# termuxinator/html5-canvas-raytracer

Hardware: AMD Instinct MI355X
Metric: Mpixel/s (higher is better)
Workload: dtype f64; 1 GPU; cfg3: h8 scene (8 spheres, 2 lights, depth 3, supersample 1) at 3840x2160; SCENE, CAMERA AND LAUNCH TABLE RESIDENT (a static frame rendered again and again: cold_frame / new_camera_every_step are the other cases); one launch per frame; kernel=fma

## Files before the change

html5-canvas-raytracer_amd/csrc/rt_kernel_math.h:

```cpp

struct v3 { double x, y, z; };
__device__ __forceinline__ v3 mk(double x, double y, double z) { v3 r; r.x = x; r.y = y; r.z = z; return r; }
__device__ __forceinline__ double dot(const v3 a, const v3 b) { return a.x * b.x + a.y * b.y + a.z * b.z; }

#if RT_STRICT
__device__ __forceinline__ double rt_sqrt(double x) { return sqrt(x); }
template <bool FMIN = false> __device__ __forceinline__ double rt_sqrt_nn(double x) { return sqrt(x); }
__device__ __forceinline__ double rt_rcp(double x) { return 1.0 / x; }
__device__ __forceinline__ double rt_div(double a, double b) { return a / b; }
__device__ __forceinline__ double rt_pow(double x, double e) { return pow(x, e); }
#define RT_DIV_CONST(x, c) ((x) / (c))
__device__ __forceinline__ v3 unit(const v3 v, double *len_out) {
  const double l = sqrt(dot(v, v));
  *len_out = l;
  if (l != 0.0) { const double s = 1.0 / l; return mk(v.x * s, v.y * s, v.z * s); }
  return v;
}
#else
__device__ __forceinline__ double rt_rsqrt_pos(double m) {
  const double y = __builtin_amdgcn_rsq(m);
  const double e = __builtin_fma(-(m * y), y, 1.0);
  return __builtin_fma(0.5 * y, e, y);
}
__device__ __forceinline__ double rt_sqrt(double x) {
  const double y = rt_rsqrt_pos(x);
  double g = x * y;
  g = __builtin_fma(__builtin_fma(-g, g, x), 0.5 * y, g);
  return (x > 0.0) ? g : x;
}
template <bool FMIN = false>
__device__ __forceinline__ double rt_sqrt_nn(double x) {
  double y;
  if constexpr (FMIN) y = __builtin_fmin(__builtin_amdgcn_rsq(x), 1e100);
  else {
    const unsigned long long yb = __builtin_bit_cast(unsigned long long, __builtin_amdgcn_rsq(x));
    const int32_t yh = (int32_t)(yb >> 32);
    y = __builtin_bit_cast(double, ((unsigned long long)(uint32_t)(yh < 0x7fe00000 ? yh : 0x7fe00000) << 32) | (uint32_t)yb);
  }
  const double e = __builtin_fma(-(x * y), y, 1.0);
  y = __builtin_fma(0.5 * y, e, y);
  const double g = x * y;
  return __builtin_fma(__builtin_fma(-g, g, x), 0.5 * y, g);
}
__device__ __forceinline__ double rt_rcp(double x) {
  double y = __builtin_amdgcn_rcp(x);
  y = __builtin_fma(y, __builtin_fma(-x, y, 1.0), y);
  return __builtin_fma(y, __builtin_fma(-x, y, 1.0), y);
}
__device__ __forceinline__ double rt_div(double a, double b) {
  const double r = rt_rcp(b);
  const double q = a * r;
  return __builtin_fma(__builtin_fma(-q, b, a), r, q);
}
#define RT_DIV_CONST(x, c) rt_div_const((x), (c), 1.0 / (c))
__device__ __forceinline__ double rt_div_const(double a, double c, double rc) {
  const double q = a * rc;
  return __builtin_fma(__builtin_fma(-q, c, a), rc, q);
}
__device__ __attribute__((noinline)) double rt_pow_generic(double x, double e) { return pow(x, e); }
template <bool UNI = false, class EP>
__device__ __forceinline__ double rt_pow_spec(double x, int32_t n, EP e) {
  const int32_t n0 = UNI ? n : __builtin_amdgcn_readfirstlane(n);
  if (UNI || __ballot(n != n0) == 0ull) {
    if (n0 < 0) return rt_pow_generic(x, *e);
    uint32_t k = (uint32_t)n0;
    if (k == 0u) return 1.0;
    double b = x;
    uint32_t g = __builtin_ctz(k);
    for (uint32_t i = 0; i < g; i++) b *= b;
    double r = b;
    for (k >>= g + 1u; k != 0u; k >>= g + 1u) {
      g = __builtin_ctz(k);
      for (uint32_t i = 0; i <= g; i++) b *= b;
      r *= b;
    }
    return r;
  }
  if (n < 0) return rt_pow_generic(x, *e);
  double r = 1.0, b = x;
  uint32_t k = (uint32_t)n;
  do { if (k & 1u) r *= b; b *= b; k >>= 1; } while (__ballot(k != 0u) != 0ull);
  return r;
}
__device__ __forceinline__ v3 unit(const v3 v, double *len_out) {
  const double m = dot(v, v);
  const double s = rt_rsqrt_pos(m);
  const bool ok = (m > 0.0);
  *len_out = ok ? m * s : m;
  return ok ? mk(v.x * s, v.y * s, v.z * s) : v;
}
#endif

#if RT_STRICT
#include "rt_fdlibm.h"
template <bool FMIN = false> __device__ __forceinline__ void rt_atan2_asin(double y, double x, double w, double *at, double *as) { *at = fd_atan2(y, x); *as = fd_asin(w); }
#else
__device__ __forceinline__ double rt_fma_k(double a, double b, double k) {
  double r;
  asm("v_fma_f64 %0, %1, %2, %3" : "=v"(r) : "v"(a), "v"(b), "s"(k));
  return r;
}
typedef const double __attribute__((address_space(4))) *rt_trig_kptr;
typedef double __attribute__((ext_vector_type(4))) rt_d4;
#define RT_TRIG_AHEAD 2u
__constant__ unsigned long long RT_TRIG_BITS[32] = {
    0x3eeba404b5e68a13ull, 0xbf23e260bd3237f4ull, 0x3f4b2bb069efb384ull, 0xbf67952daf56de9bull,
    0x3f7d6d43a595c56full, 0xbf8c6ea4a57d9582ull, 0x3f967e295f08b19full, 0xbf9e9ae6fc27006aull,
    0x3fa2c15b5711927aull, 0x3fa059859fea6a70ull, 0xbfa59976e82d3ff0ull, 0xbf90a5a378a05eafull,
    0x3fa82d5d6ef28734ull, 0x3f94052137024d6aull, 0xbfaae5ce6a214619ull, 0x3f7ab3a098a70509ull,
    0x3fae1bb48427b883ull, 0x3f88ed60a300c8d2ull, 0xbfb110e48b207f05ull, 0x3f8c6fa84b77012bull,
    0x3fb3b13657b87036ull, 0x3f91c6c111dccb70ull, 0xbfb745d119378e4full, 0x3f96e89f0a0adacfull,
    0x3fbc71c717e1913cull, 0x3f9f1c72c668963full, 0xbfc2492492376b7dull, 0x3fa6db6db41ce4bdull,
    0x3fc99999999952ccull, 0x3fb333333336fd5bull, 0xbfd5555555555523ull, 0x3fc5555555555380ull};
template <bool FMIN = false>
__device__ __forceinline__ void rt_atan2_asin(double y, double x, double w, double *at, double *as) {
  rt_trig_kptr K = (rt_trig_kptr)(const void *)RT_TRIG_BITS;
  asm volatile("" : "+s"(K));
#define RT_TRIG_GROUP(I) (*(const rt_d4 __attribute__((address_space(4))) *)(K + 4 * (I)))
  rt_d4 g[8];
  g[0] = RT_TRIG_GROUP(0); g[1] = RT_TRIG_GROUP(1);
  const double ax = __builtin_fabs(x), ay = __builtin_fabs(y);
  const double hi = __builtin_fmax(ax, ay), lo = __builtin_fmin(ax, ay);
  const double q = rt_div(lo, hi);
  const double z = q * q;
  const double yw = __builtin_fabs(w);
  const double t = __builtin_fma(yw, -0.5, 0.5);
  const bool big = (yw >= 0.5);
  const double r = big ? t : w * w;
  g[2] = RT_TRIG_GROUP(2);
  double p = g[0][0];
  p = rt_fma_k(p, z, g[0][1]); p = rt_fma_k(p, z, g[0][2]); p = rt_fma_k(p, z, g[0][3]);
  g[3] = RT_TRIG_GROUP(3);
  p = rt_fma_k(p, z, g[1][0]); p = rt_fma_k(p, z, g[1][1]); p = rt_fma_k(p, z, g[1][2]); p = rt_fma_k(p, z, g[1][3]);
  double pa = 0.0;
#pragma unroll
  for (uint32_t i = 2; i < 8; i++) {
    if (i + RT_TRIG_AHEAD < 8u) g[i + RT_TRIG_AHEAD] = RT_TRIG_GROUP(i + RT_TRIG_AHEAD);
    p = rt_fma_k(p, z, g[i][0]);
    pa = (i == 2u) ? g[i][1] : rt_fma_k(pa, r, g[i][1]);
    p = rt_fma_k(p, z, g[i][2]);
    pa = rt_fma_k(pa, r, g[i][3]);
  }
#undef RT_TRIG_GROUP
  double a = __builtin_fma(q, z * p, q);
  a = (ay > ax) ? (M_PI / 2.0 - a) : a;
  const bool xneg = (__builtin_bit_cast(unsigned long long, x) >> 63) != 0;
  a = xneg ? (M_PI - a) : a;
  a = (hi == 0.0) ? (xneg ? M_PI : 0.0) : a;
  *at = __builtin_copysign(a, y);
  pa = pa * r;
  const double sq = big ? rt_sqrt_nn<FMIN>(t) : yw;
  const double ww = __builtin_fma(sq, pa, sq);
  double b = big ? __builtin_fma(-2.0, ww, M_PI / 2.0) : ww;
  b = (yw > 1.0) ? __builtin_nan("") : b;
  *as = __builtin_copysign(b, w);
}
#endif

__device__ __forceinline__ v3 reflect(const v3 v, const v3 n) {
  const double t = -(2.0 * dot(v, n));
  return mk(v.x + n.x * t, v.y + n.y * t, v.z + n.z * t);
}
__device__ __forceinline__ double min1(double x) { return (x > 1.0) ? 1.0 : x; }
__device__ __forceinline__ double maxa(double a, double x) { return (x < a) ? a : x; }

__device__ __forceinline__ uint32_t lowbias32(uint32_t x) {
  x ^= x >> 16; x *= 0x7feb352du; x ^= x >> 15; x *= 0x846ca68bu; x ^= x >> 16;
  return x;
}
__device__ __forceinline__ double star_uniform(uint32_t pix_lo, uint32_t pix_hi, uint32_t path, uint32_t mix) {
  return (double)lowbias32(pix_lo ^ lowbias32(path + 0x9e3779b9u * ((pix_hi ^ mix) + 1u))) * (1.0 / 4294967296.0);
}

__device__ __forceinline__ int to_int32_bit0(double x) {
  if (fabs(x) < 2147483648.0) return (int)x & 1;
  if (!(fabs(x) < RT_INF)) return 0;
  double t = trunc(x);
  if (fabs(t) >= 4294967296.0) t = t - floor(t / 4294967296.0) * 4294967296.0;
  return (int)((long long)t & 1);
}

__device__ __forceinline__ uint32_t to_byte(double c) {
#if RT_STRICT
  return (uint32_t)__builtin_rint(__builtin_fmin(__builtin_fmax(255.0 * c, 0.0), 255.0));
#else
  const double s = __builtin_fmin(__builtin_fmax(255.0 * c, 0.0), 255.0) + 6755399441055744.0;
  return (uint32_t)__builtin_bit_cast(unsigned long long, s);
#endif
}
```

html5-canvas-raytracer_amd/csrc/rt_kernel_trace.h:

```cpp

#define RT_PIN() asm volatile("")
#define RT_ROOT(TCA, DISC)                                                                    \
        const double thc_ = rt_sqrt_nn<REFRACT>(DISC);                                                 \
        const double t0_ = (TCA) - thc_, t1_ = (TCA) + thc_;                                  \
        const bool in_ = (t0_ < eps);                                                         \
        const double t_ = in_ ? t1_ : t0_;
#define RT_CAND(IDX, TCA, DISC)                                                               \
      if (!((DISC) < 0.0)) {                                                                  \
        RT_PIN();                                                                             \
        RT_ROOT(TCA, DISC)                                                                    \
        const bool closer_ = (t_ < ht) && !(t_ < eps);              \
        ht = closer_ ? t_ : ht;                                                               \
        hcode = closer_ ? ((int)(2u * (IDX)) + (in_ ? 1 : 0)) : hcode;                        \
      }
#define RT_GENERIC(IDX, G)                                                                    \
      {                                                                                       \
        const v3 Lv_ = mk((G).ox - p.x, (G).oy - p.y, (G).oz - p.z);                          \
        const double tca_ = dot(d, Lv_);                                                      \
        const double disc_ = (G).r2 - (dot(Lv_, Lv_) - tca_ * tca_);                          \
        RT_CAND(IDX, tca_, disc_)                                                             \
      }
#define RT_ANCHORED_DISC(G)                                                                   \
        const double tca_ = d.x * (G).ox + d.y * (G).oy + d.z * (G).oz;                       \
        const double disc_ = __builtin_fma(tca_, tca_, -(G).r2);
#define RT_ANCHORED(IDX, G)                                                                   \
      {                                                                                       \
        RT_ANCHORED_DISC(G)                                                                   \
        RT_CAND(IDX, tca_, disc_)                                                             \
      }

#if !RT_STRICT
__device__ __forceinline__ float rt_q_of(float qp, float x, float c, float rp_over_r) {
  const float ic = __builtin_amdgcn_rcpf(fmaxf(c, 1e-30f));
  return fminf(ic * (qp * (6.f * x + rp_over_r) + x + 0.5f * x * x) + x, 1e30f);
}
__device__ __forceinline__ int rt_lvl(int lv) { return lv & 255; }
#define RT_Q_GET(L_) __builtin_bit_cast(float, (uint32_t)(L_) & 0xffff0000u)
__device__ __forceinline__ int rt_q_put(int lv, float q) { return (int)(((uint32_t)lv & 0xffffu) | ((__builtin_bit_cast(uint32_t, q) + 0xffffu) & 0xffff0000u)); }
__device__ __forceinline__ float rt_r_get(int lv) { return __builtin_bit_cast(float, ((uint32_t)lv & 0xff00u) << 15); }
__device__ __forceinline__ int rt_r_put(int lv, float r) { return (int)(((uint32_t)lv & 0xffff00ffu) | ((((__builtin_bit_cast(uint32_t, r) >> 23) + 1u) & 255u) << 8)); }
constexpr float RT_Q_FLAT = 4096.f;
#define RT_Q_OF(QP, T, INVR, C, RP) rt_q_of((QP), (T) * (INVR), (C), (RP) * (INVR))
#else
__device__ __forceinline__ int rt_lvl(int lv) { return lv; }
#endif

#if !RT_STRICT
#define RT_XY_INDEX(XU, XV, FU, FV)                                                                                \
          const unsigned long long su = __builtin_bit_cast(unsigned long long, (XU) + 6442450944.0), sv = __builtin_bit_cast(unsigned long long, (XV) + 6442450944.0);   \
          uint32_t iu = __builtin_amdgcn_alignbit((uint32_t)(su >> 32), (uint32_t)su, 20u) ^ 0x80000000u;        \
          uint32_t iv = __builtin_amdgcn_alignbit((uint32_t)(sv >> 32), (uint32_t)sv, 20u) ^ 0x80000000u;       \
           \
          const bool near_ = (min(((uint32_t)su + 1u) & 0xfffffu, ((uint32_t)sv + 1u) & 0xfffffu) <= 2u);           \
           \
          if constexpr (UNI) { if (__ballot(near_) != 0ull) return false; }                                    \
          if (!UNI && near_) {                                                                                  \
            RT_PIN();                                                                                             \
            iu = (uint32_t)(XU); iv = (uint32_t)(XV);                    \
            const rt_launch __attribute__((address_space(4))) *K = rt_cold_args();                                \
             \
            float q_here = RT_Q_GET(level);                                                                        \
            if (rt_lvl(level) == 0 && q_here == 0.f) {                   \
              const float ex = (float)(h.x - K->cam_origin[0]), ey = (float)(h.y - K->cam_origin[1]), ez = (float)(h.z - K->cam_origin[2]);   \
              q_here = RT_Q_OF(0.f, __builtin_sqrtf(ex * ex + ey * ey + ez * ez), (float)m.inv_r, __builtin_fabsf((float)dot(d, n)), 0.f);       \
            }                                                                                                     \
            double tol = (K->mark_flags & RT_MARK_ALL) ? 2.0 : K->flag_tol * (double)fmaxf(1.f, q_here * (1.f / RT_Q_FLAT));   \
                          \
            if ((K->mark_flags & (RT_MARK_WEIGHT | RT_MARK_ALL)) == RT_MARK_WEIGHT) {                              \
              double S_ = map_valid ? acc[0] : 1.0;                                                               \
              if constexpr (FOLD_FORWARD && REFRACT) for (int i_ = 0; i_ < sp; i_++) S_ *= (parked[i_].map_valid ? parked[i_].S : 1.0) * parked[i_].a3;   \
              if (__builtin_fabs(S_) * 510.0 < 0.9) tol = -1.0;                                                    \
            }                                                                                                     \
             \
            const bool zf = !(K->mark_flags & RT_MARK_ZERO);                                                       \
            const bool bu = (zf && (FU) == 0.0 && (XU) == 0.0) || (__builtin_fabs((XU) - __builtin_rint(XU)) >= tol);    \
            const bool bv = (zf && (FV) == 0.0 && (XV) == 0.0) || (__builtin_fabs((XV) - __builtin_rint(XV)) >= tol);    \
            if (!(bu & bv)) {                                                                                      \
              uint32_t t3 = threadIdx.x;                                                                          \
              asm volatile("" : "+v"(t3));                                                                        \
              rt_mark_append<SS2>(rt_pixel_of<SS2, W1>(L, t3));                                                        \
            }                                                                                                     \
          }
#endif

#if !RT_STRICT
#define RT_SDISC(G, TC, DISC)                                                                 \
            const double TC = -(sv.x * (G).ox + sv.y * (G).oy + sv.z * (G).oz);               \
            const double DISC = __builtin_fma(TC, TC, -(G).r2);
#define RT_SROOTS(TC, THC, T0, T1) const double T0 = llen - (TC + THC), T1 = llen - (TC - THC);
#else
#define RT_SDISC(G, TC, DISC)                                                                 \
            const v3 Lv_ = mk((G).ox - h.x, (G).oy - h.y, (G).oz - h.z);                      \
            const double TC = dot(sv, Lv_);                                                   \
            const double DISC = (G).r2 - (dot(Lv_, Lv_) - TC * TC);
#define RT_SROOTS(TC, THC, T0, T1) const double T0 = TC - THC, T1 = TC + THC;
#endif
#define RT_SHADOW(J, G)                                                                       \
            {                                                                                 \
              const bool other_ = ((int)(J) != hi);                                           \
              if (COUNT && other_ && !blocked) tests++;                                       \
              RT_SDISC(G, tc_, disc_)                                                         \
              if (other_ && !(disc_ < 0.0) && !blocked) {                                     \
                RT_PIN();                                                                     \
                const double thc_ = rt_sqrt_nn<REFRACT>(disc_);                                        \
                RT_SROOTS(tc_, thc_, t0_, t1_)                                                \
                const double t_ = (t0_ < eps) ? t1_ : t0_;                                    \
                if ((t_ < llen) && !(t_ < eps)) {                                             \
                  RT_PIN();                                                                   \
                  const double oa4_ = objs[J].albedo[4];                                      \
                  if (oa4_ != 0.0) li = rt_div(li, oa4_);    \
                  else { li = 0.0; blocked = true; }                                          \
                }                                                                             \
              }                                                                               \
            }
#define RT_SHADOW_U(J, G)                                                                     \
            {                                                                               \
              RT_SDISC(G, tc_, disc_)                                                       \
              if (((int)(J) != hi) && !(disc_ < 0.0)) {                                     \
                RT_PIN();                                                                   \
                const double thc_ = rt_sqrt_nn<REFRACT>(disc_);                                      \
                RT_SROOTS(tc_, thc_, t0_, t1_)                                              \
                const double t_ = (t0_ < eps) ? t1_ : t0_;                                  \
                if ((t_ < llen) && !(t_ < eps) && li != 0.0) {                              \
                  RT_PIN();                                                                 \
                  const double oa4_ = objs[J].albedo[4];                                    \
                  li = (oa4_ != 0.0) ? rt_div(li, oa4_) : 0.0;                              \
                }                                                                           \
              }                                                                             \
            }

template <bool REFRACT, bool COUNT, bool GRID, bool SS2, bool ITEM = false, bool W1 = false, bool UNI = false>
__device__ __forceinline__ bool trace_pixel(const rt_launch &L, const rt_mtl *mtl, const rt_texture_desc *tex,
                                            [[maybe_unused]] double *acc, [[maybe_unused]] const rt_geom *cull_lds, [[maybe_unused]] const rt_geom cull0, [[maybe_unused]] uint32_t lane,
                                            [[maybe_unused]] double blk_x0, [[maybe_unused]] double blk_x1, [[maybe_unused]] double blk_y0,
                                            [[maybe_unused]] double blk_y1, v3 p, v3 d, double rgb[3], uint32_t cnt[3],
                                            [[maybe_unused]] bool is_probe, [[maybe_unused]] uint32_t cand_host,
                                            [[maybe_unused]] uint32_t own_sx = 0u, [[maybe_unused]] uint32_t own_sy = 0u, [[maybe_unused]] uint32_t own_f = 0u) {
  static_assert(!UNI || (W1 && !REFRACT && !COUNT && !ITEM && !RT_STRICT), "uniform-material path: the one-wave-workgroup product kernels");
#ifdef RT_TESTING
  uint32_t probe_n = 0;
  double probe_li = 0.0;
#endif
  const sphere_kptr objs = (sphere_kptr)L.objects;
  const geom_kptr geom = (geom_kptr)L.geom;
  const uint32_t N = L.n_objects, NL = L.n_lights;
  const double eps = L.epsilon;
  const uint32_t NLOOP = L.n_loop;
  const uint32_t enc = L.enclosing;
  const bool cull_lds_on = (!RT_STRICT && !COUNT) ? !GRID : (L.cull_in_lds != 0u);
#if RT_STRICT
  constexpr bool FOLD_FORWARD = false;
#else
  constexpr bool FOLD_FORWARD = true;
#endif
  [[maybe_unused]] frame<REFRACT> stack[FOLD_FORWARD ? 1 : RT_MAX_SEGS];
  [[maybe_unused]] park parked[(FOLD_FORWARD && REFRACT) ? RT_MAX_SEGS : 1];
  [[maybe_unused]] int sp = 0;
  [[maybe_unused]] bool map_valid = false;
  int level = 0;
  [[maybe_unused]] uint32_t tree_path = 1u;
#if defined(RT_TESTING) && defined(RT_ABLATE_BOUNCE)
  uint32_t segs_left = L.segs ? 1 : 0;
#else
  uint32_t segs_left = L.segs;
#endif
  double ret[3] = {0.0, 0.0, 0.0};

  double ht = RT_INF; int hcode = -1;
  if constexpr (UNI) { if (segs_left == 0) return false; }
  if (segs_left != 0) {
        [[maybe_unused]] const geom_kptr ga = (geom_kptr)L.geom_cam;
#if !RT_STRICT
        if constexpr (UNI) {
          const uint32_t i = cand_host & 255u;
          const rt_geom g0 = rt_load_geom32(ga, i);
          typename rt_mtl_src<true>::type &mu = *rt_mtl_at<true>(mtl, i);
          if ((mu.albedo[3] > 0.0 && segs_left > 1) || rt_mtl_kind(mu) == RT_SAMPLER_STARS) return false;
          RT_ANCHORED_DISC(g0)
          RT_ROOT(tca_, disc_)
          const bool met_ = !(disc_ < 0.0) && (t_ < ht) && !(t_ < eps);
          if (__ballot(!met_) != 0ull) return false;
#if defined(RT_TESTING) && defined(RT_ABLATE_UNIFORM)
          rgb[0] = rgb[1] = rgb[2] = 0.0;
          return true;
#endif
          ht = t_; hcode = (int)(2u * i) + (in_ ? 1 : 0);
        } else
        if (cand_host != 0u) {
          { const uint32_t i = cand_host & 255u; const rt_geom g0 = rt_load_geom32(ga, i); RT_ANCHORED(i, g0) }
          if (cand_host >= (2u << 16)) { const uint32_t i = (cand_host >> 8) & 255u; const rt_geom g0 = rt_load_geom32(ga, i); RT_ANCHORED(i, g0) }
        } else
#endif
        for (uint32_t base = 0; base < NLOOP; base += 64u) {
          const uint32_t j = base + lane;
          const uint32_t jj = j < NLOOP ? j : 0u;
          double c0 = cull0.ox, c1 = cull0.oy, c2 = cull0.oz, c3 = cull0.r2;
          if constexpr (ITEM) {
          } else if (cull_lds_on) {
            const rt_geom __attribute__((address_space(3))) *g = (const rt_geom __attribute__((address_space(3))) *)cull_lds + jj;
            c0 = g->ox; c1 = g->oy; c2 = g->oz; c3 = g->r2;
          } else if (base != 0u) {
            const rt_geom __attribute__((address_space(1))) *g = (const rt_geom __attribute__((address_space(1))) *)L.cull + jj;
            c0 = g->ox; c1 = g->oy; c2 = g->oz; c3 = g->r2;
          }
          const rt_geom cr = rt_geom{c0, c1, c2, c3};
          unsigned long long m = __ballot(j < NLOOP) & __ballot(cr.ox * L.proj_d <= blk_x1) & __ballot(cr.oy * L.proj_d >= blk_x0) &
                                 __ballot(cr.oz * L.proj_d <= blk_y1) & __ballot(cr.r2 * L.proj_d >= blk_y0);
          if constexpr (ITEM) m = (NLOOP - base >= 64u) ? ~0ull : ((1ull << (NLOOP - base)) - 1ull);
          while (m) {
            const uint32_t i = base + (uint32_t)__builtin_ctzll(m);
            m &= m - 1ull;
#if RT_STRICT
            const rt_geom g0 = rt_load_geom32(geom, i);
            RT_GENERIC(i, g0)
#else
            const rt_geom g0 = rt_load_geom32(ga, i);
            RT_ANCHORED(i, g0)
#endif
          }
        }
  }
  bool searched = true;
  [[maybe_unused]] bool first_bounce = false;
#if !RT_STRICT
  if (!UNI && L.sky_fast && segs_left != 0 && __ballot(hcode >= 0) == 0ull) {
    if (COUNT) { cnt[0]++; cnt[2] += N; }
    rgb[0] = L.sky_rgb[0]; rgb[1] = L.sky_rgb[1]; rgb[2] = L.sky_rgb[2];
    return true;
  }
#endif

  if (segs_left != 0) {
    for (;;) {
      if (COUNT) cnt[0]++;
      if (!UNI && !searched) {
        bool scanned = false;
#if !RT_STRICT
        if constexpr (GRID) {
          if (rt_cold_args()->bounce_table != nullptr) {
            const uint32_t from = (uint32_t)(hcode >> 1);
            const double ax = __builtin_fabs(d.x), ay = __builtin_fabs(d.y), az = __builtin_fabs(d.z);
            const bool bx = (ax >= ay) && (ax >= az), by = !bx && (ay >= az);
            const double dm = bx ? d.x : (by ? d.y : d.z);
            const double du = bx ? d.y : d.x, dv = (bx || by) ? d.z : d.y;
            const double sc = (0.5 * RT_BGRID) * __builtin_amdgcn_rcp(__builtin_fabs(dm));
            const double fu = __builtin_fmin(__builtin_fmax(__builtin_fma(du, sc, 0.5 * RT_BGRID), 0.0), (double)(RT_BGRID - 1u));
            const double fv = __builtin_fmin(__builtin_fmax(__builtin_fma(dv, sc, 0.5 * RT_BGRID), 0.0), (double)(RT_BGRID - 1u));
            const uint32_t face = (bx ? 0u : (by ? 2u : 4u)) + ((dm < 0.0) ? 1u : 0u);
            const uint32_t key = from * RT_BCELLS + face * (RT_BGRID * RT_BGRID) + (uint32_t)fv * RT_BGRID + (uint32_t)fu;
            const uint32_t words = (NLOOP + 63u) >> 6;
            ht = RT_INF; hcode = -1;
            for (uint32_t wd = 0; wd < words; wd++) {
              unsigned long long cand = 0ull, todo = __ballot(true);
              uint32_t distinct = 0;
              while (todo) {
                const uint32_t k0 = (uint32_t)__builtin_amdgcn_readlane((int)key, (int)__builtin_ctzll(todo));
                cand |= rt_load_word32(rt_cold_args()->bounce_table, k0 * words + wd);
                todo &= ~__ballot(key == k0);
                if (++distinct == 16u && todo) {
                  cand = (wd + 1u == words && (NLOOP & 63u)) ? ((1ull << (NLOOP & 63u)) - 1ull) : ~0ull;
                  break;
                }
              }
              while (cand) {
                const uint32_t j = (wd << 6) + (uint32_t)__builtin_ctzll(cand);
                cand &= cand - 1ull;
                const rt_geom g0 = rt_load_geom32(geom, j);
                RT_GENERIC(j, g0)
              }
            }
            scanned = true;
          }
        }
#endif
#if !RT_STRICT
        if constexpr (!GRID && !REFRACT && !COUNT && !ITEM) {
          if (first_bounce) {
            uint32_t fb = rt_entry_first_bounce<W1>(L);
#ifdef RT_TESTING
            if (L.no_first_bounce) fb = 0u;
#endif
            if (fb >> 31) {
              ht = RT_INF; hcode = -1;
              uint32_t m = (fb >> RT_CELL_SHIFT) & ((1u << RT_FB_MAX_LOOP) - 1u);
              uint32_t sn = rt_entry_second_node<W1>(L);
#ifdef RT_TESTING
              if (L.no_second_node) sn = 0u;
              if ((sn & (RT_SN_SELF0 | RT_SN_SELF1)) && L.uniform_waves != nullptr && __builtin_ctzll(__ballot(true)) == (int)lane) atomicAdd(L.uniform_waves + 3, 1ull);
#endif
              if (sn & RT_SN_SELF0) m &= ~(1u << (fb & 255u));
              if (sn & RT_SN_SELF1) m &= ~(1u << ((fb >> 8) & 255u));
              while (m) {
                const uint32_t i = (uint32_t)__builtin_ctz(m);
                m &= m - 1u;
                const rt_geom g0 = rt_load_geom32(geom, i);
                RT_GENERIC(i, g0)
              }
              scanned = true;
#ifdef RT_TESTING
              if (L.uniform_waves != nullptr && __builtin_ctzll(__ballot(true)) == (int)lane) atomicAdd(L.uniform_waves + 2, 1ull);
#endif
            }
          }
        }
#endif
        if (!scanned) {
          ht = RT_INF; hcode = -1;
          uint32_t i = 0;
          for (; i + 2 <= NLOOP; i += 2) {
            const rt_geom_pair gp = rt_load_geom_pair32(geom, i);
            const rt_geom g0 = gp.a, g1 = gp.b;
            RT_GENERIC(i, g0) RT_GENERIC(i + 1, g1)
          }
          if (i < NLOOP) { const rt_geom g0 = rt_load_geom32(geom, i); RT_GENERIC(i, g0) }
        }
      }
      [[maybe_unused]] const bool primary_node = UNI || searched;
      first_bounce = searched;
      searched = false;
      if (!UNI && enc != ~0u && hcode < 0) {
        if (L.enclosing_flat) {
          ht = 1.0; hcode = (int)(2u * enc + 1u);
        } else {
          const rt_geom g0 = rt_load_geom32(geom, enc);
          RT_GENERIC(enc, g0)
        }
      }
      if (COUNT) cnt[2] += N;
      const int hi = UNI ? (int)(cand_host & 255u) : (hcode >> 1);
      const bool inside = (hcode & 1) != 0;
      bool descend = false;
#if defined(RT_TESTING) && defined(RT_ABLATE_SHADE)
      if (true) { ret[0] = ht; ret[1] = (double)hcode; ret[2] = 0.0; } else
#endif
      if (!UNI && hcode < 0) {
        { const auto &mc = RT_COLD(miss_color); ret[0] = mc[0]; ret[1] = mc[1]; ret[2] = mc[2]; }
#ifdef RT_TESTING
        if (is_probe && probe_n < RT_PROBE_NODES) {
          double *q = L.probe + (size_t)(probe_n++) * RT_PROBE_WORDS;
          for (uint32_t z = 0; z < RT_PROBE_WORDS; z++) q[z] = 0.0;
          q[0] = (double)(REFRACT ? tree_path : (1u << rt_lvl(level))); q[1] = -1.0; q[2] = ht; q[9] = d.x; q[10] = d.y; q[11] = d.z;
          q[17] = (double)segs_left; q[19] = p.x; q[20] = p.y; q[21] = p.z; q[23] = 1.0;
        }
#endif
      } else {
        typename rt_mtl_src<UNI>::type &m = *rt_mtl_at<UNI>(mtl, (uint32_t)hi);
        const v3 h = mk(p.x + d.x * ht, p.y + d.y * ht, p.z + d.z * ht);
#if RT_STRICT
        double nlen;
        const v3 n = unit(mk(h.x - m.origin[0], h.y - m.origin[1], h.z - m.origin[2]), &nlen);
#else
        const double inv_r = m.inv_r;
        const v3 n = mk((h.x - m.origin[0]) * inv_r, (h.y - m.origin[1]) * inv_r, (h.z - m.origin[2]) * inv_r);
#endif
        v3 l;
        if (UNI && __ballot(inside) == 0ull) l = n;
        else l = inside ? mk(-n.x, -n.y, -n.z) : n;
        const double a0 = m.albedo[0], a1 = m.albedo[1], a2 = m.albedo[2], a3 = m.albedo[3];
        const double a4 = REFRACT ? m.albedo[4] : 0.0;
#if !RT_STRICT && !defined(RT_ABLATE_QAMP)
        if (!UNI && (rt_lvl(level) != 0 || ((a3 > 0.0 || a4 > 0.0) && segs_left > 1))) {
          const float ir_ = (float)inv_r;
          const float q_ = RT_Q_OF(RT_Q_GET(level), (float)ht, ir_, __builtin_fabsf((float)dot(d, n)), rt_r_get(level));
          level = rt_q_put(level, q_);
          level = rt_r_put(level, __builtin_amdgcn_rcpf(ir_));
        }
#endif

        double col[3];
#if defined(RT_TESTING) && defined(RT_ABLATE_SAMPLER)
        const int kind = RT_SAMPLER_COLOR;
#else
        const int kind = rt_mtl_kind(m);
#endif
#if RT_STRICT
        if (kind == RT_SAMPLER_TEXTURE) {
          double t_at, t_as;
          rt_atan2_asin<REFRACT>(-n.z, -n.x, -n.y, &t_at, &t_as);
          const double u = RT_DIV_CONST(t_at, M_PI) / 2.0 + 0.5;
          const double v = RT_DIV_CONST(t_as, M_PI / 2.0) / 2.0 + 0.5;
          const rt_texture_desc td = rt_tex_desc<UNI>(tex, rt_mtl_texture(m));
          const double xd = ceil(u * (double)td.width) - 1.0, yd = ceil(v * (double)td.height) - 1.0;
          uint32_t xi = (xd > 0.0) ? (uint32_t)xd : 0u, yi = (yd > 0.0) ? (uint32_t)yd : 0u;
          xi = min(xi, td.width - 1u); yi = min(yi, td.height - 1u);
          const uint32_t texel = *(const uint32_t *)(L.texel_base + td.texels_offset + ((size_t)yi * td.width + xi) * 4u);
          col[0] = RT_DIV_CONST((double)(texel & 255u), 255.0); col[1] = RT_DIV_CONST((double)((texel >> 8) & 255u), 255.0);
          col[2] = RT_DIV_CONST((double)((texel >> 16) & 255u), 255.0);
          if (xd != xd || yd != yd) col[0] = col[1] = col[2] = __builtin_nan("");
        } else if (kind == RT_SAMPLER_CHECKER) {
          double t_at, t_as;
          rt_atan2_asin<REFRACT>(-n.y, -n.x, -n.z, &t_at, &t_as);
          const double u = RT_DIV_CONST(t_at, M_PI) / 2.0 + 0.5;
          const double v = RT_DIV_CONST(t_as, M_PI / 2.0) / 2.0 + 0.5;
          const int c = to_int32_bit0(u * m.c[6]) ^ to_int32_bit0(v * m.c[7]);
          col[0] = m.c[3 * c]; col[1] = m.c[3 * c + 1]; col[2] = m.c[3 * c + 2];
#else
        [[maybe_unused]] double t_at, t_as;
        [[maybe_unused]] const bool one_cell = UNI && !GRID && kind == RT_SAMPLER_CHECKER && (cand_host & (1u << 24)) != 0u;
        if (UNI && one_cell) {
          const uint32_t c3 = (cand_host >> 28) & 1u ? 3u : 0u;
          col[0] = m.c[c3]; col[1] = m.c[c3 + 1u]; col[2] = m.c[c3 + 2u];
        } else if (UNI && kind != RT_SAMPLER_TEXTURE && kind != RT_SAMPLER_CHECKER) {
          col[0] = m.c[0]; col[1] = m.c[1]; col[2] = m.c[2];
        } else {
        if constexpr (UNI) {
          const bool tx_ = (kind == RT_SAMPLER_TEXTURE);
          rt_atan2_asin<REFRACT>(tx_ ? -n.z : -n.y, -n.x, tx_ ? -n.y : -n.z, &t_at, &t_as);
        }
        if (kind == RT_SAMPLER_TEXTURE) {
          if constexpr (!UNI) rt_atan2_asin<REFRACT>(-n.z, -n.x, -n.y, &t_at, &t_as);
          const double u = RT_DIV_CONST(t_at, M_PI) / 2.0 + 0.5;
          const double v = RT_DIV_CONST(t_as, M_PI / 2.0) / 2.0 + 0.5;
          const rt_texture_desc td = rt_tex_desc<UNI>(tex, rt_mtl_texture(m));
          const double xu = u * (double)td.width, xv = v * (double)td.height;
          RT_XY_INDEX(xu, xv, 1.0, 1.0)
          const uint32_t xi = min(iu, td.width - 1u), yi = min(iv, td.height - 1u);
          const uint32_t texel = *(const uint32_t *)(rt_cold_args()->texel_base + td.texels_offset + ((size_t)yi * td.width + xi) * 4u);
          col[0] = RT_DIV_CONST((double)(texel & 255u), 255.0); col[1] = RT_DIV_CONST((double)((texel >> 8) & 255u), 255.0);
          col[2] = RT_DIV_CONST((double)((texel >> 16) & 255u), 255.0);
        } else if (kind == RT_SAMPLER_CHECKER) {
          if constexpr (!UNI) rt_atan2_asin<REFRACT>(-n.y, -n.x, -n.z, &t_at, &t_as);
          const double u = RT_DIV_CONST(t_at, M_PI) / 2.0 + 0.5;
          const double v = RT_DIV_CONST(t_as, M_PI / 2.0) / 2.0 + 0.5;
          const double xu = u * m.c[6], xv = v * m.c[7];
          RT_XY_INDEX(xu, xv, m.c[6], m.c[7])
          const int c = (int)((iu ^ iv) & 1u);
          if constexpr (UNI) {
            double k0 = m.c[0], k1 = m.c[1], k2 = m.c[2], k3 = m.c[3], k4 = m.c[4], k5 = m.c[5];
            asm volatile("" : "+s"(k0), "+s"(k1), "+s"(k2), "+s"(k3), "+s"(k4), "+s"(k5));
            col[0] = c ? k3 : k0; col[1] = c ? k4 : k1; col[2] = c ? k5 : k2;
          } else { col[0] = m.c[3 * c]; col[1] = m.c[3 * c + 1]; col[2] = m.c[3 * c + 2]; }
#endif
        } else if (!UNI && kind == RT_SAMPLER_STARS) {
          uint32_t sx = own_sx, sy = own_sy, f = own_f;
          if constexpr (!ITEM) {
            f = blockIdx.z;
            uint32_t t3 = threadIdx.x;
            asm volatile("" : "+v"(t3));
            const rt_pixel P = rt_pixel_of<SS2, W1>(L, t3);
            sx = SS2 ? 2u * P.px + (P.sub & 1u) : P.px; sy = SS2 ? 2u * P.frow + (P.sub >> 1) : P.frow;
          }
          const unsigned long long pix = (unsigned long long)sy * (SS2 ? 2u * L.w : L.w) + sx;
          const uint32_t path = REFRACT ? tree_path : (1u << rt_lvl(level));
          const rt_launch __attribute__((address_space(4))) *K = rt_cold_args();
          const uint32_t mix = lowbias32(K->stars_seed + K->stars_step * f);
          double c = star_uniform((uint32_t)pix, (uint32_t)(pix >> 32), path, mix);
          c = (c >= m.c[6]) ? 0.0 : c * m.c[7];
          col[0] = col[1] = col[2] = c;
        } else { col[0] = m.c[0]; col[1] = m.c[1]; col[2] = m.c[2]; }
#if !RT_STRICT
        }
#endif

        if constexpr (FOLD_FORWARD && REFRACT) {
#pragma unroll
          for (int c = 0; c < 3; c++) acc[(10 + c) * RT_WG_THREADS] = col[c];
        }

        double diffuse = 0.0, specular = 0.0;
#if defined(RT_TESTING) && defined(RT_ABLATE_LIGHT)
        if (false) {
#else
        if (a1 > 0.0 || a2 > 0.0) {
#endif
          double li = RT_COLD(light_intensity);
#if !RT_STRICT
          [[maybe_unused]] uint32_t smask = ~0u;
          if constexpr (!COUNT) { if (primary_node) smask = rt_entry_shadow_masks<W1>(L); }
#endif
          for (uint32_t k = 0; k < NL; k++) {
            double llen;
            const double *lk = (const double *)((const char *)&L.lights[0][0] + (uint32_t)(k * 24u));
#if !RT_STRICT
            [[maybe_unused]] rt_geom_pair gp_first;
            if constexpr (!GRID && !COUNT) {
              [[maybe_unused]] const geom_kptr gl = (geom_kptr)L.geom_light;
              gp_first = rt_load_geom_pair32(gl, k * L.n_objects);
            }
#endif
            const v3 sraw = mk(lk[0] - h.x, lk[1] - h.y, lk[2] - h.z);
            const double lmag = dot(sraw, sraw);
#if RT_STRICT
            const v3 sv = unit(sraw, &llen);
#else
            const double inv_llen = rt_rsqrt_pos(lmag);
            llen = lmag * inv_llen;
            const v3 sv = mk(sraw.x * inv_llen, sraw.y * inv_llen, sraw.z * inv_llen);
#endif
            const double sdot = dot(sv, l);
#if RT_STRICT
            if (sdot <= 0.0) continue;
#else
            if (!(sdot > 0.0)) continue;
#endif
            if (COUNT) cnt[1]++;
            uint32_t tests = 0;
            bool blocked = false;
#if !RT_STRICT
            const geom_kptr gl = (geom_kptr)L.geom_light;
            const uint32_t glo = k * L.n_objects;
#else
            const geom_kptr gl = geom;
            const uint32_t glo = 0u;
#endif
#if defined(RT_TESTING) && defined(RT_ABLATE_SHADOW)
            const uint32_t NS = 0;
#elif defined(RT_TESTING) && defined(RT_ABLATE_SHADOW4)
            const uint32_t NS = NLOOP > 4u ? NLOOP - 4u : NLOOP;
#else
            const uint32_t NS = NLOOP;
#endif
#if !RT_STRICT
            bool no_occluder = false;
            if constexpr (!COUNT) no_occluder = primary_node && k < 2u && ((smask >> (16u * k)) & 0xffffu) == 0u;
            if (no_occluder) {
            } else
            if (GRID && rt_cold_args()->shadow_grid != nullptr && li != 0.0) {
              const void *const sgrid = rt_cold_args()->shadow_grid;
              const double __attribute__((address_space(4))) *gh = (const double __attribute__((address_space(4))) *)sgrid + 16u * k;
              const v3 vv = mk(-sraw.x, -sraw.y, -sraw.z);
              const double vx = gh[0] * vv.x + gh[1] * vv.y + gh[2] * vv.z, vy = gh[3] * vv.x + gh[4] * vv.y + gh[5] * vv.z;
              const double vz = gh[6] * vv.x + gh[7] * vv.y + gh[8] * vv.z;
              const double iz = rt_rcp(vz);
              const double fx = __builtin_fmin(__builtin_fmax((vx * iz - gh[9]) * gh[11], 0.0), (double)(RT_SGRID - 1));
              const double fy = __builtin_fmin(__builtin_fmax((vy * iz - gh[10]) * gh[12], 0.0), (double)(RT_SGRID - 1));
              const bool proj = (vz > 0.0) && (fx == fx) && (fy == fy);
              const uint32_t cell = proj ? (uint32_t)fy * RT_SGRID + (uint32_t)fx : (uint32_t)(RT_SGRID * RT_SGRID);
              const uint32_t words = (NLOOP + 63u) >> 6;
              const uint32_t cells_at = 16u * NL + k * (RT_SGRID * RT_SGRID + 1u) * words;
              for (uint32_t wd = 0; wd < words; wd++) {
                unsigned long long cand = 0ull, todo = __ballot(true);
                while (todo) {
                  const uint32_t c0 = (uint32_t)__builtin_amdgcn_readlane((int)cell, (int)__builtin_ctzll(todo));
                  cand |= rt_load_word32(sgrid, cells_at + c0 * words + wd);
                  todo &= ~__ballot(cell == c0);
                }
                while (cand) {
                  const uint32_t j = (wd << 6) + (uint32_t)__builtin_ctzll(cand);
                  cand &= cand - 1ull;
                  const rt_geom g0 = rt_load_geom32(gl, glo + j);
                  RT_SHADOW_U(j, g0)
                }
              }
            } else
#endif
            if (!COUNT) {
              if constexpr (UNI) RT_PIN();
              if (li != 0.0) {
                uint32_t j = 0;
#if !RT_STRICT
                [[maybe_unused]] uint32_t mk = ~0u;
                if constexpr (!GRID) { if (primary_node && k < 2u) mk = (smask >> (16u * k)) | 0xffff0000u; }
                if constexpr (!GRID) {
                  if (NS >= 2u) { if (mk & 3u) { const rt_geom g0 = gp_first.a, g1 = gp_first.b; RT_SHADOW_U(0u, g0) RT_SHADOW_U(1u, g1) } j = 2u; }
                }
#endif
                for (; j + 2 <= NS; j += 2) {
#if !RT_STRICT
                  if (!GRID && j < 31u && ((mk >> j) & 3u) == 0u) continue;
#endif
                  const rt_geom_pair gp = rt_load_geom_pair32(gl, glo + j);
                  const rt_geom g0 = gp.a, g1 = gp.b;
                  RT_SHADOW_U(j, g0) RT_SHADOW_U(j + 1, g1)
                }
#if !RT_STRICT
                if (j < NS && (GRID || j >= 32u || ((mk >> j) & 1u))) { const rt_geom g0 = rt_load_geom32(gl, glo + j); RT_SHADOW_U(j, g0) }
#else
                if (j < NS) { const rt_geom g0 = rt_load_geom32(gl, glo + j); RT_SHADOW_U(j, g0) }
#endif
              }
            } else
            if (COUNT || li != 0.0) {
              uint32_t j = 0;
              for (; j + 2 <= NS; j += 2) {
                const rt_geom g0 = rt_load_geom32(gl, glo + j), g1 = rt_load_geom32(gl, glo + j + 1);
                RT_SHADOW(j, g0) RT_SHADOW(j + 1, g1)
                if (blocked) break;
              }
              if (j < NS && !blocked) { const rt_geom g0 = rt_load_geom32(gl, glo + j); RT_SHADOW(j, g0) }
            }
            if (COUNT) cnt[2] += tests;
            if (li == 0.0) continue;
#if RT_STRICT
            diffuse += li * sdot / lmag;
#else
            diffuse += (li * sdot) * (inv_llen * inv_llen);
#endif
#if defined(RT_TESTING) && defined(RT_ABLATE_SPEC)
            if (false) {
#else
            if (a2 > 0.0) {
#endif
#if RT_STRICT
              double ql;
              const v3 q = unit(reflect(mk(-sv.x, -sv.y, -sv.z), l), &ql);
              const double spd = d.x * -q.x + d.y * -q.y + d.z * -q.z;
#else
              const double t2 = 2.0 * sdot;
              const v3 q = mk(__builtin_fma(l.x, t2, -sv.x), __builtin_fma(l.y, t2, -sv.y), __builtin_fma(l.z, t2, -sv.z));
              const double spd = -(d.x * q.x + d.y * q.y + d.z * q.z);
#endif
#if !RT_STRICT
              typename rt_mtl_src<UNI>::type *spec_m = &m;
              if constexpr (GRID && !REFRACT && !COUNT && !UNI) {
                uint32_t off_ = (uint32_t)hi * (uint32_t)sizeof(rt_mtl);
                asm volatile("" : "+v"(off_));
                spec_m = (const rt_mtl *)((const char *)mtl + off_);
              }
              const int32_t spec_n = spec_m->spec_n;
              if (spd > 0.0) specular += rt_pow_spec<UNI>(spd, spec_n, &spec_m->specular_exponent);
#else
              if (spd > 0.0) specular += rt_pow(spd, m.specular_exponent);
#endif
            }
          }
          diffuse = min1(diffuse) * a1;
          specular = min1(specular) * a2;
#ifdef RT_TESTING
          probe_li = li;
#endif
        }

#if RT_STRICT
        const v3 nq = n;
#else
        const v3 nq = inside ? mk(-l.x, -l.y, -l.z) : l;
#endif
        v3 r = mk(0, 0, 0); double rlen = 0.0;
        if (!UNI && a3 > 0.0 && segs_left > 1) r = unit(reflect(d, nq), &rlen);
        v3 f = mk(0, 0, 0); double flen = 0.0;
        if (REFRACT && a4 > 0.0 && segs_left > 1) {
          const double dn = dot(d, nq);
          double cosi = -((dn < -1.0) ? -1.0 : min1(dn));
          v3 nn = nq; double eta;
          if (cosi < 0.0) { cosi = -cosi; nn = mk(-nq.x, -nq.y, -nq.z); eta = m.refract_index; }
          else eta = rt_rcp(m.refract_index);
          const double k = 1.0 - eta * eta * (1.0 - cosi * cosi);
          if (k > 0.0) {
            const double q = eta * cosi - rt_sqrt(k);
            f = mk(d.x * eta + nn.x * q, d.y * eta + nn.y * q, d.z * eta + nn.z * q);
          } else f = reflect(d, nn);
          f = unit(f, &flen);
        }

        if constexpr (FOLD_FORWARD && REFRACT) {
#pragma unroll
          for (int c = 0; c < 3; c++) col[c] = acc[(10 + c) * RT_WG_THREADS];
        }
        const bool go_r = !UNI && (rlen != 0.0);
        const bool go_f = REFRACT && (flen != 0.0);
#ifdef RT_TESTING
        if (is_probe && probe_n < RT_PROBE_NODES) {
          double *q = L.probe + (size_t)(probe_n++) * RT_PROBE_WORDS;
          q[0] = (double)(REFRACT ? tree_path : (1u << rt_lvl(level))); q[1] = (double)hcode; q[2] = ht;
          q[3] = h.x; q[4] = h.y; q[5] = h.z; q[6] = n.x; q[7] = n.y; q[8] = n.z; q[9] = d.x; q[10] = d.y; q[11] = d.z;
          q[12] = col[0]; q[13] = col[1]; q[14] = col[2]; q[15] = diffuse; q[16] = specular; q[17] = (double)segs_left;
          q[18] = probe_li; q[19] = p.x; q[20] = p.y; q[21] = p.z; q[22] = (double)(go_r ? 1 : 0) + 2.0 * (go_f ? 1 : 0); q[23] = 1.0;
        }
#endif
        if (!go_r && !go_f) {
#pragma unroll
          for (int c = 0; c < 3; c++) ret[c] = maxa(col[c] * a0, min1(col[c] * diffuse + col[c] * specular));
        } else if constexpr (FOLD_FORWARD) {
          const uint32_t T = W1 ? 64u : RT_WG_THREADS;
          double A[3], D[3];
#pragma unroll
          for (int c = 0; c < 3; c++) { A[c] = col[c] * a0; D[c] = col[c] * diffuse + col[c] * specular; }
          const bool via_f = REFRACT && !go_r;
          if (REFRACT && go_r && go_f) {
            park &pk = parked[sp++];
#pragma unroll
            for (int c = 0; c < 3; c++) { pk.amb[c] = A[c]; pk.ds[c] = D[c]; }
            pk.a3 = a3; pk.a4 = a4; pk.h[0] = h.x; pk.h[1] = h.y; pk.h[2] = h.z; pk.f[0] = f.x; pk.f[1] = f.y; pk.f[2] = f.z;
            pk.path = tree_path; pk.segs_left = segs_left; pk.level = level; pk.map_valid = map_valid; pk.hcode = hcode;
            if (map_valid) {
              pk.S = acc[0];
#pragma unroll
              for (int c = 0; c < 3; c++) { pk.O[c] = acc[(1 + c) * T]; pk.LO[c] = acc[(4 + c) * T]; pk.HI[c] = acc[(7 + c) * T]; }
            }
            map_valid = false;
            p = h; d = r; tree_path = 2u * tree_path;
          } else {
            const double coef = via_f ? a4 : a3;
            if (!map_valid) {
              acc[0] = coef;
#pragma unroll
              for (int c = 0; c < 3; c++) { acc[(1 + c) * T] = D[c]; acc[(4 + c) * T] = A[c]; acc[(7 + c) * T] = __builtin_fmax(A[c], 1.0); }
            } else {
              const double S = acc[0];
#pragma unroll
              for (int c = 0; c < 3; c++) {
                const double O = acc[(1 + c) * T], LO = acc[(4 + c) * T], HI = acc[(7 + c) * T];
                const double l2 = __builtin_fma(S, A[c], O), h2 = __builtin_fma(S, __builtin_fmax(A[c], 1.0), O);
                acc[(1 + c) * T] = __builtin_fma(S, D[c], O);
                acc[(4 + c) * T] = __builtin_fmax(LO, __builtin_fmin(HI, l2));
                acc[(7 + c) * T] = __builtin_fmax(LO, __builtin_fmin(HI, h2));
              }
              acc[0] = S * coef;
            }
            map_valid = true;
            p = h; d = via_f ? f : r; tree_path = 2u * tree_path + (via_f ? 1u : 0u);
          }
          level++; segs_left--;
          descend = true;
        } else {
          frame<REFRACT> &fr = stack[level];
#pragma unroll
          for (int c = 0; c < 3; c++) { fr.amb[c] = col[c] * a0; fr.ds[c] = col[c] * diffuse + col[c] * specular; }
          fr.a3 = a3;
          if constexpr (REFRACT) {
            fr.a4 = a4; fr.h[0] = h.x; fr.h[1] = h.y; fr.h[2] = h.z; fr.f[0] = f.x; fr.f[1] = f.y; fr.f[2] = f.z;
            fr.re[0] = fr.re[1] = fr.re[2] = 0.0;
            fr.has_f = go_f; fr.phase = go_r ? 0 : 1;
          }
          p = h; d = go_r ? r : f;
          tree_path = 2u * tree_path + (go_r ? 0u : 1u);
          level++; segs_left--;
          descend = true;
        }
      }
      if (descend) continue;

      if constexpr (FOLD_FORWARD) {
        const uint32_t T = W1 ? 64u : RT_WG_THREADS;
        if (map_valid) {
          const double S = acc[0];
#pragma unroll
          for (int c = 0; c < 3; c++) ret[c] = __builtin_fmax(acc[(4 + c) * T], __builtin_fmin(acc[(7 + c) * T], __builtin_fma(S, ret[c], acc[(1 + c) * T])));
        }
        bool resumed = false;
        if constexpr (REFRACT) {
          if (sp > 0) {
            const park &pk = parked[--sp];
            const double coef = pk.a4;
            if (!pk.map_valid) {
              acc[0] = coef;
#pragma unroll
              for (int c = 0; c < 3; c++) {
                acc[(1 + c) * T] = pk.ds[c] + ret[c] * pk.a3; acc[(4 + c) * T] = pk.amb[c]; acc[(7 + c) * T] = __builtin_fmax(pk.amb[c], 1.0);
              }
            } else {
              const double S = pk.S;
#pragma unroll
              for (int c = 0; c < 3; c++) {
                const double Dn = pk.ds[c] + ret[c] * pk.a3;
                const double l2 = __builtin_fma(S, pk.amb[c], pk.O[c]), h2 = __builtin_fma(S, __builtin_fmax(pk.amb[c], 1.0), pk.O[c]);
                acc[(1 + c) * T] = __builtin_fma(S, Dn, pk.O[c]);
                acc[(4 + c) * T] = __builtin_fmax(pk.LO[c], __builtin_fmin(pk.HI[c], l2));
                acc[(7 + c) * T] = __builtin_fmax(pk.LO[c], __builtin_fmin(pk.HI[c], h2));
              }
              acc[0] = S * coef;
            }
            map_valid = true;
            p = mk(pk.h[0], pk.h[1], pk.h[2]); d = mk(pk.f[0], pk.f[1], pk.f[2]);
            tree_path = 2u * pk.path + 1u; segs_left = pk.segs_left - 1u; level = pk.level + 1;
            hcode = pk.hcode;

            resumed = true;
          }
        }
        if (!resumed) break;
      } else {
        bool resumed = false;
        while (level > 0) {
          level--; segs_left++; tree_path >>= 1;
          frame<REFRACT> &fr = stack[level];
          if constexpr (REFRACT) {
            if (fr.phase == 0) {
              fr.re[0] = ret[0] * fr.a3; fr.re[1] = ret[1] * fr.a3; fr.re[2] = ret[2] * fr.a3;
              if (fr.has_f) {
                fr.phase = 1;
                p = mk(fr.h[0], fr.h[1], fr.h[2]); d = mk(fr.f[0], fr.f[1], fr.f[2]);
                tree_path = 2u * tree_path + 1u;
                level++; segs_left--;
                resumed = true;
                break;
              }
#pragma unroll
              for (int c = 0; c < 3; c++) ret[c] = maxa(fr.amb[c], min1(fr.ds[c] + fr.re[c]));
            } else {
#pragma unroll
              for (int c = 0; c < 3; c++) ret[c] = maxa(fr.amb[c], min1(fr.ds[c] + fr.re[c] + ret[c] * fr.a4));
            }
          } else {
#pragma unroll
            for (int c = 0; c < 3; c++) ret[c] = maxa(fr.amb[c], min1(fr.ds[c] + ret[c] * fr.a3));
          }
        }
        if (!resumed) break;
      }
    }
  }
  rgb[0] = ret[0]; rgb[1] = ret[1]; rgb[2] = ret[2];
  return true;
}

#undef RT_Q_GET
#undef RT_Q_OF
#undef RT_ROOT
#undef RT_CAND
#undef RT_GENERIC
#undef RT_ANCHORED_DISC
#undef RT_ANCHORED
#undef RT_XY_INDEX
#undef RT_SDISC
#undef RT_SROOTS
#undef RT_SHADOW
#undef RT_SHADOW_U
```

Baseline: 155,400 Mpixel/s.

## Use raw v_min/v_max asm and drop redundant checks on the uniform non-refract path

Replaces fmin/fmax (which emit extra canonicalization ops for NaN handling) with inline v_min_f64/v_max_f64 asm in the lean non-refract fold path and shading clamp. The uniform-hit shortcut drops the inside-sphere root selection and the inside ballot, and reflection uses an unguarded normalize. A wavefront-wide NaN ballot falls back to the exact clamp when any lane produces NaN, to keep NaN semantics. This cuts ALU instructions in the inner shading loop, but it assumes a uniform hit never comes from inside a sphere and relies on hardware min/max NaN behavior.

```diff
diff --git a/html5-canvas-raytracer_amd/csrc/rt_kernel_math.h b/html5-canvas-raytracer_amd/csrc/rt_kernel_math.h
--- a/html5-canvas-raytracer_amd/csrc/rt_kernel_math.h
+++ b/html5-canvas-raytracer_amd/csrc/rt_kernel_math.h
@@ -163,6 +163,18 @@
 }
 __device__ __forceinline__ double min1(double x) { return (x > 1.0) ? 1.0 : x; }
 __device__ __forceinline__ double maxa(double a, double x) { return (x < a) ? a : x; }
+__device__ __forceinline__ double rt_min_nn(double a, double b) { double r; asm("v_min_f64 %0, %1, %2" : "=v"(r) : "v"(a), "v"(b)); return r; }
+__device__ __forceinline__ double rt_max_nn(double a, double b) { double r; asm("v_max_f64 %0, %1, %2" : "=v"(r) : "v"(a), "v"(b)); return r; }
+__device__ __forceinline__ double rt_min1_nn(double x) { double r; asm("v_min_f64 %0, %1, 1.0" : "=v"(r) : "v"(x)); return r; }
+__device__ __forceinline__ double rt_max1_nn(double x) { double r; asm("v_max_f64 %0, %1, 1.0" : "=v"(r) : "v"(x)); return r; }
+#if !RT_STRICT
+__device__ __forceinline__ v3 unit_go(const v3 v, double *len_out) {
+  const double m = dot(v, v);
+  const double s = rt_rsqrt_pos(m);
+  *len_out = (m > 0.0) ? m * s : m;
+  return mk(v.x * s, v.y * s, v.z * s);
+}
+#endif
 
 __device__ __forceinline__ uint32_t lowbias32(uint32_t x) {
   x ^= x >> 16; x *= 0x7feb352du; x ^= x >> 15; x *= 0x846ca68bu; x ^= x >> 16;
diff --git a/html5-canvas-raytracer_amd/csrc/rt_kernel_trace.h b/html5-canvas-raytracer_amd/csrc/rt_kernel_trace.h
--- a/html5-canvas-raytracer_amd/csrc/rt_kernel_trace.h
+++ b/html5-canvas-raytracer_amd/csrc/rt_kernel_trace.h
@@ -153,6 +153,7 @@
 #else
   constexpr bool FOLD_FORWARD = true;
 #endif
+  constexpr bool LEAN = !RT_STRICT && !REFRACT && !COUNT && !ITEM;
   [[maybe_unused]] frame<REFRACT> stack[FOLD_FORWARD ? 1 : RT_MAX_SEGS];
   [[maybe_unused]] park parked[(FOLD_FORWARD && REFRACT) ? RT_MAX_SEGS : 1];
   [[maybe_unused]] int sp = 0;
@@ -177,14 +178,14 @@
           typename rt_mtl_src<true>::type &mu = *rt_mtl_at<true>(mtl, i);
           if ((mu.albedo[3] > 0.0 && segs_left > 1) || rt_mtl_kind(mu) == RT_SAMPLER_STARS) return false;
           RT_ANCHORED_DISC(g0)
-          RT_ROOT(tca_, disc_)
-          const bool met_ = !(disc_ < 0.0) && (t_ < ht) && !(t_ < eps);
+          const double t0_ = tca_ - rt_sqrt_nn<REFRACT>(disc_);
+          const bool met_ = !(disc_ < 0.0) && (t0_ < ht) && !(t0_ < eps);
           if (__ballot(!met_) != 0ull) return false;
 #if defined(RT_TESTING) && defined(RT_ABLATE_UNIFORM)
           rgb[0] = rgb[1] = rgb[2] = 0.0;
           return true;
 #endif
-          ht = t_; hcode = (int)(2u * i) + (in_ ? 1 : 0);
+          ht = t0_; hcode = (int)(2u * i);
         } else
         if (cand_host != 0u) {
           { const uint32_t i = cand_host & 255u; const rt_geom g0 = rt_load_geom32(ga, i); RT_ANCHORED(i, g0) }
@@ -354,7 +355,7 @@
         const v3 n = mk((h.x - m.origin[0]) * inv_r, (h.y - m.origin[1]) * inv_r, (h.z - m.origin[2]) * inv_r);
 #endif
         v3 l;
-        if (UNI && __ballot(inside) == 0ull) l = n;
+        if constexpr (UNI) l = n;
         else l = inside ? mk(-n.x, -n.y, -n.z) : n;
         const double a0 = m.albedo[0], a1 = m.albedo[1], a2 = m.albedo[2], a3 = m.albedo[3];
         const double a4 = REFRACT ? m.albedo[4] : 0.0;
@@ -458,6 +459,7 @@
         }
 
         double diffuse = 0.0, specular = 0.0;
+        [[maybe_unused]] double draw = 0.0, sraw = 0.0;
 #if defined(RT_TESTING) && defined(RT_ABLATE_LIGHT)
         if (false) {
 #else
@@ -614,8 +616,14 @@
 #endif
             }
           }
+          if constexpr (UNI) {
+            draw = diffuse; sraw = specular;
+            diffuse = rt_min1_nn(diffuse) * a1;
+            specular = rt_min1_nn(specular) * a2;
+          } else {
           diffuse = min1(diffuse) * a1;
           specular = min1(specular) * a2;
+          }
 #ifdef RT_TESTING
           probe_li = li;
 #endif
@@ -627,6 +635,9 @@
         const v3 nq = inside ? mk(-l.x, -l.y, -l.z) : l;
 #endif
         v3 r = mk(0, 0, 0); double rlen = 0.0;
+#if !RT_STRICT
+        if constexpr (LEAN) { if (!UNI && a3 > 0.0 && segs_left > 1) r = unit_go(reflect(d, l), &rlen); } else
+#endif
         if (!UNI && a3 > 0.0 && segs_left > 1) r = unit(reflect(d, nq), &rlen);
         v3 f = mk(0, 0, 0); double flen = 0.0;
         if (REFRACT && a4 > 0.0 && segs_left > 1) {
@@ -659,6 +670,25 @@
         }
 #endif
         if (!go_r && !go_f) {
+          if constexpr (UNI) {
+            double x[3];
+#pragma unroll
+            for (int c = 0; c < 3; c++) x[c] = col[c] * diffuse + col[c] * specular;
+            const double poison = (((draw + sraw) + x[0]) + x[1]) + x[2];
+            if (__ballot(poison != poison) == 0ull) {
+#pragma unroll
+              for (int c = 0; c < 3; c++) ret[c] = rt_max_nn(col[c] * a0, rt_min1_nn(x[c]));
+            } else {
+#if defined(RT_TESTING) && defined(RT_ABLATE_LIGHT)
+              const bool lit = false;
+#else
+              const bool lit = (a1 > 0.0 || a2 > 0.0);
+#endif
+              const double d2 = lit ? min1(draw) * a1 : 0.0, s2 = lit ? min1(sraw) * a2 : 0.0;
+#pragma unroll
+              for (int c = 0; c < 3; c++) ret[c] = maxa(col[c] * a0, min1(col[c] * d2 + col[c] * s2));
+            }
+          } else
 #pragma unroll
           for (int c = 0; c < 3; c++) ret[c] = maxa(col[c] * a0, min1(col[c] * diffuse + col[c] * specular));
         } else if constexpr (FOLD_FORWARD) {
@@ -685,16 +715,23 @@
             if (!map_valid) {
               acc[0] = coef;
 #pragma unroll
-              for (int c = 0; c < 3; c++) { acc[(1 + c) * T] = D[c]; acc[(4 + c) * T] = A[c]; acc[(7 + c) * T] = __builtin_fmax(A[c], 1.0); }
+              for (int c = 0; c < 3; c++) { acc[(1 + c) * T] = D[c]; acc[(4 + c) * T] = A[c]; acc[(7 + c) * T] = LEAN ? rt_max1_nn(A[c]) : __builtin_fmax(A[c], 1.0); }
             } else {
               const double S = acc[0];
 #pragma unroll
               for (int c = 0; c < 3; c++) {
                 const double O = acc[(1 + c) * T], LO = acc[(4 + c) * T], HI = acc[(7 + c) * T];
+                if constexpr (LEAN) {
+                  const double l2 = __builtin_fma(S, A[c], O), h2 = __builtin_fma(S, rt_max1_nn(A[c]), O);
+                  acc[(1 + c) * T] = __builtin_fma(S, D[c], O);
+                  acc[(4 + c) * T] = rt_max_nn(LO, rt_min_nn(HI, l2));
+                  acc[(7 + c) * T] = rt_max_nn(LO, rt_min_nn(HI, h2));
+                } else {
                 const double l2 = __builtin_fma(S, A[c], O), h2 = __builtin_fma(S, __builtin_fmax(A[c], 1.0), O);
                 acc[(1 + c) * T] = __builtin_fma(S, D[c], O);
                 acc[(4 + c) * T] = __builtin_fmax(LO, __builtin_fmin(HI, l2));
                 acc[(7 + c) * T] = __builtin_fmax(LO, __builtin_fmin(HI, h2));
+                }
               }
               acc[0] = S * coef;
             }
@@ -726,7 +763,10 @@
         if (map_valid) {
           const double S = acc[0];
 #pragma unroll
-          for (int c = 0; c < 3; c++) ret[c] = __builtin_fmax(acc[(4 + c) * T], __builtin_fmin(acc[(7 + c) * T], __builtin_fma(S, ret[c], acc[(1 + c) * T])));
+          for (int c = 0; c < 3; c++) {
+            if constexpr (LEAN) ret[c] = rt_max_nn(acc[(4 + c) * T], rt_min_nn(acc[(7 + c) * T], __builtin_fma(S, ret[c], acc[(1 + c) * T])));
+            else ret[c] = __builtin_fmax(acc[(4 + c) * T], __builtin_fmin(acc[(7 + c) * T], __builtin_fma(S, ret[c], acc[(1 + c) * T])));
+          }
         }
         bool resumed = false;
         if constexpr (REFRACT) {
```

New measurement: 160,000 Mpixel/s (median of 6 runs). +3.0%, better.
